# CarluerJB/3D_SIFT_CUDA

Measured on AMD Instinct MI355X. Metric: keypoints/s (.key records per second; Gauss-pyramid GB/s vs HBM roofline in `pyramid`/`roofline`), higher is better.
Workload: dtype f32; 1 GPU; 512^3 float32 blob-field volume per GPU, full featExtract path (pyramid + DoG + extrema + keypoints + SIFT-rank descriptor), all octaves; records_per_volume=185421, octaves=8, extrema=43900, keypoints=36792, parallelism=single GPU, tuning=defaults, descriptor_parity=SIFT-rank: pinned against the reference (see DESIGN.md section 2)

## Files before the change

3d_sift_cuda_amd/csrc/api_slab.hip:

```cpp
#include <algorithm>
#include <chrono>
#include <cmath>
#include <cstdarg>
#include <cstdio>
#include <cstdlib>
#include <cstring>
#include <vector>

#include "sift3d_internal.h"

#include "pipeline.h"

extern "C" int sift3d_candidates_reset(sift3d_ctx *c)
{
    if (!c) return SIFT3D_ERR_ARG;
    HIPCHK(c, hipSetDevice(c->device));
    timing_begin(c);
    return cand_reset(c);
}

extern "C" int sift3d_extrema_append_dev(sift3d_ctx *c, const float *d_prev, const float *d_cur, const float *d_next,
                                         int64_t nx, int64_t ny, int64_t nz_local, int level_id, int64_t z_lo, int64_t z_hi)
{
    if (!c || !d_prev || !d_cur || !d_next) return SIFT3D_ERR_ARG;
// ... 5 lines not shown
    if (rc) return rc;
    rc = cand_append(c, {d_prev, d_cur, d_next, nx, ny, nz_local, (int)z_lo, (int)z_hi, level_id}, cand_where(), true);
    if (rc) return rc;
    return fence_out(c);
}

extern "C" int sift3d_lazy_levels_supported(int64_t nx, int64_t ny, int64_t nz_local, float next_sigma)
{
    float taps[SIFT3D_MAX_TAPS];
    return lazy_shape_ok(nx, ny, nz_local) && sift3d_gauss_taps(next_sigma, 0.01f, taps) == 2 * SIFT3D_FAST_MAX_R + 1 ? 1 : 0;
}

extern "C" int sift3d_extrema_append_lazy_dev(sift3d_ctx *c, const float *d_prev, const float *g_prev_a, const float *g_prev_b,
                                              const float *d_cur, const float *d_next, const float *g_next, float next_sigma,
                                              int64_t nx, int64_t ny, int64_t nz_local, int level_id, int64_t z_lo, int64_t z_hi)
{
    if (!c || !d_cur || (!d_prev && !(g_prev_a && g_prev_b)) || (!d_next && !g_next)) return SIFT3D_ERR_ARG;
    if (nx <= 0 || ny <= 0 || nz_local <= 0 || nx >= (1ll << 31) || ny >= (1ll << 31) || nz_local >= 65538 ||
        nx * ny * nz_local > (int64_t)SIFT3D_KEY_IDX_MASK || level_id < 0 || level_id >= 96)
        return set_err(c, SIFT3D_ERR_ARG, "bad extrema_append arguments");
    float taps[SIFT3D_MAX_TAPS];
    const int ntaps = d_next ? 0 : sift3d_gauss_taps(next_sigma, 0.01f, taps);
    if (((!d_prev || !d_next) && !lazy_shape_ok(nx, ny, nz_local)) || (!d_next && ntaps != 2 * SIFT3D_FAST_MAX_R + 1))
        return set_err(c, SIFT3D_ERR_ARG, "this shape or filter needs stored DoG levels (sift3d_lazy_levels_supported)");
    HIPCHK(c, hipSetDevice(c->device));
    int rc = fence_in(c);
    if (rc) return rc;
    level_job jb = {d_prev ? d_prev : g_prev_a, d_cur, d_next, nx, ny, nz_local, (int)z_lo, (int)z_hi, level_id};
    if (!d_prev) jb.prev_b = g_prev_b;
    if (!d_next) {
        jb.next_ntaps = ntaps;
        for (int q = 0; q < ntaps; q++) jb.next_taps[q] = taps[q];
        jb.next_g = g_next;
    }
    rc = cand_append(c, jb, cand_where(), true);
    if (rc) return rc;
    return fence_out(c);
}

static int levels_from_desc(sift3d_ctx *c, const sift3d_level_desc *ld, int n, std::vector<sift3d_level> &levels)
{
    if (!ld || n <= 0 || n > 96) return set_err(c, SIFT3D_ERR_ARG, "bad level table");
    levels.resize((size_t)n);
    for (int i = 0; i < n; i++) {
        sift3d_level &lv = levels[(size_t)i];
        lv.img = ld[i].img;
        lv.XP = (int)ld[i].nx;
        lv.dogc = ld[i].dogc;
        lv.X = (int)ld[i].nx; lv.Y = (int)ld[i].ny; lv.Z = (int)ld[i].nz_global;
        lv.Zl = (int)ld[i].nz_local;
        lv.z_off = (int)ld[i].z_offset;
        lv.sigma_h = ld[i].sigma_h; lv.sigma_c = ld[i].sigma_c; lv.sigma_l = ld[i].sigma_l;
        lv.octave_factor = ld[i].octave_factor;
        lv.pad = 0;
    }
    return SIFT3D_OK;
}

extern "C" int sift3d_candidates_dev(sift3d_ctx *c, const sift3d_level_desc *levels, int n_levels, sift3d_candidate **out,
                                     int64_t *n_out)
{
    if (!c || !out || !n_out) return SIFT3D_ERR_ARG;
    HIPCHK(c, hipSetDevice(c->device));
    std::vector<sift3d_level> lv;
    int rc = levels_from_desc(c, levels, n_levels, lv);
    if (rc) return rc;
    rc = fence_in(c);
    if (rc) return rc;
    int64_t ncand = 0;
    rc = cand_finalize(c, &ncand);
    if (rc) return rc;
    return candidates_to_host(c, lv, ncand, out, n_out);
}

extern "C" int sift3d_describe_dev(sift3d_ctx *c, const sift3d_level_desc *levels, int n_levels, int desc_mode,
                                   float eig_thres, float size_factor, const sift3d_feature **view, const int32_t **group_view,
                                   int64_t *n_out)
{
    if (!c || !view || !n_out) return SIFT3D_ERR_ARG;
    if (desc_mode < SIFT3D_DESC_SIFT || desc_mode > SIFT3D_DESC_NRRIEF) return set_err(c, SIFT3D_ERR_ARG, "bad descriptor mode");
    HIPCHK(c, hipSetDevice(c->device));
    std::vector<sift3d_level> lv;
    int rc = levels_from_desc(c, levels, n_levels, lv);
    if (rc) return rc;
    rc = fence_in(c);
    if (rc) return rc;
    int64_t ncand = 0;
    rc = cand_finalize(c, &ncand);
    if (rc) return rc;
    c->last.n_extrema = ncand;
    rc = describe_sorted(c, lv, ncand, desc_mode, eig_thres, size_factor, n_out);
    if (rc) return rc;
    *view = c->h_recs;
    if (group_view) *group_view = c->h_group;
    return SIFT3D_OK;
}

extern "C" int sift3d_describe_dev_counts(sift3d_ctx *c, const sift3d_level_desc *levels, int n_levels, int desc_mode, float eig_thres,
                                          float size_factor, const int32_t **group_counts, int64_t *n_records)
{
    if (!c || !group_counts || !n_records) return SIFT3D_ERR_ARG;
    if (desc_mode < SIFT3D_DESC_SIFT || desc_mode > SIFT3D_DESC_NRRIEF) return set_err(c, SIFT3D_ERR_ARG, "bad descriptor mode");
    HIPCHK(c, hipSetDevice(c->device));
    std::vector<sift3d_level> lv;
    int rc = levels_from_desc(c, levels, n_levels, lv);
    if (rc) return rc;
    rc = fence_in(c);
// ... 99 lines not shown
```

3d_sift_cuda_amd/csrc/desc_bins.h:

```cpp
#ifndef DESC_BINS_H
#define DESC_BINS_H

#if defined(__HIPCC__) || defined(__CUDACC__)
#define DESC_BINS_HD __host__ __device__
#else
#define DESC_BINS_HD
#endif
#if defined(__clang__)
#define DESC_BINS_UNROLL _Pragma("unroll")
#define DESC_BINS_ROLLED _Pragma("nounroll")
#else
#define DESC_BINS_UNROLL
#define DESC_BINS_ROLLED
#endif

#define DESC_BINS_PD 11
#define DESC_BINS_NI 9
#define DESC_BINS_NINT 729
#define DESC_BINS_BOX 5
#define DESC_BINS_NONE 8
#define DESC_BINS_ZS 83
#define DESC_BINS_LEN (DESC_BINS_NI * DESC_BINS_ZS)

DESC_BINS_HD constexpr float desc_bins_floor_ce(float x) { return (float)(int)x > x ? (float)((int)x - 1) : (float)(int)x; }

DESC_BINS_HD constexpr void interp_coord(float fX, float fMin, float fMax, int &ix, float &w)
{
    if (fX < fMin + 0.5f) {
        ix = (int)fMin;
        w = 1.0f;
    } else if (fX >= fMax - 0.5f) {
        ix = (int)(fMax - 2);
        w = 0.0f;
    } else {
        float mh = fX - 0.5f;
        ix = (int)(__builtin_is_constant_evaluated() ? desc_bins_floor_ce(mh) : __builtin_floorf(mh));
        w = 1.0f - (mh - ((float)ix));
    }
}

DESC_BINS_HD constexpr float desc_bins_weight(int b, int c)
{
    const float binsz = DESC_BINS_PD / (float)2;
    float v = (int)(c / binsz) + 0.5f;
    if ((int)((c + 0) / binsz) != (int)((c + 1) / binsz)) {
        float p0 = ((c + 0) / binsz);
        float p1 = ((c + 1) / binsz);
        v = (p0 + p1) / 2.0f;
    }
    float w = 0;
    int i0 = 0;
    interp_coord(v, 0, 2.0f, i0, w);
    return b ? 1.0f - w : w;
}
static_assert(desc_bins_weight(0, 1) == 1 && desc_bins_weight(0, 2) == 1 && desc_bins_weight(0, 3) == 1 && desc_bins_weight(0, 4) == 1 &&
                  desc_bins_weight(1, 1) == 0 && desc_bins_weight(1, 2) == 0 && desc_bins_weight(1, 3) == 0 && desc_bins_weight(1, 4) == 0,
              "patch coordinates 1 .. 4 belong to bin 0 alone");
static_assert(desc_bins_weight(0, 5) == 0.5f && desc_bins_weight(1, 5) == 0.5f, "the centre plane is shared in halves");
static_assert(desc_bins_weight(0, 6) == 0 && desc_bins_weight(0, 7) == 0 && desc_bins_weight(0, 8) == 0 && desc_bins_weight(0, 9) == 0 &&
                  desc_bins_weight(1, 6) == 1 && desc_bins_weight(1, 7) == 1 && desc_bins_weight(1, 8) == 1 && desc_bins_weight(1, 9) == 1,
              "patch coordinates 6 .. 9 belong to bin 1 alone");

DESC_BINS_HD constexpr int desc_bins_octant(int lane) { return lane & 7; }
DESC_BINS_HD constexpr int desc_bins_axis_bin(int lane, int axis) { return (lane >> (3 + axis)) & 1; }
DESC_BINS_HD constexpr int desc_bins_origin(int b) { return b ? DESC_BINS_BOX : 1; }
DESC_BINS_HD constexpr int desc_bins_entry(int x, int y, int z) { return (z - 1) * DESC_BINS_ZS + (y - 1) * DESC_BINS_NI + (x - 1); }

DESC_BINS_HD constexpr bool desc_bins_needs_all(float mg) { return mg == __builtin_huge_valf(); }

DESC_BINS_HD inline void desc_bins_box_weights(int b, float *w)
{
    DESC_BINS_UNROLL
    for (int d = 0; d < DESC_BINS_BOX; d++) w[d] = b ? desc_bins_weight(1, desc_bins_origin(1) + d) : desc_bins_weight(0, desc_bins_origin(0) + d);
}

DESC_BINS_HD inline float desc_bins_walk(const float *mag, const unsigned char *bin, int lane)
{
    const int o = desc_bins_octant(lane);
    const int bx = desc_bins_axis_bin(lane, 0), by = desc_bins_axis_bin(lane, 1), bz = desc_bins_axis_bin(lane, 2);
    float wx[DESC_BINS_BOX], wy[DESC_BINS_BOX], wz[DESC_BINS_BOX];
    desc_bins_box_weights(bx, wx);
    desc_bins_box_weights(by, wy);
    desc_bins_box_weights(bz, wz);
    const int base = desc_bins_entry(desc_bins_origin(bx), desc_bins_origin(by), desc_bins_origin(bz));
    mag += base;
    bin += base;
    float acc = 0;
    DESC_BINS_UNROLL
    for (int dz = 0; dz < DESC_BINS_BOX; dz++) {
        DESC_BINS_UNROLL
        for (int dy = 0; dy < DESC_BINS_BOX; dy++) {
// ... 30 lines not shown
```

3d_sift_cuda_amd/csrc/kernels_keypoint.hip:

```cpp
#include <cstddef>
#include <type_traits>

#include "desc_bins.h"
#include "sift3d_internal.h"

#define PD SIFT3D_PATCH_DIM
#define PV SIFT3D_PATCH_VOX



__device__ __forceinline__ float trilinear(const float *__restrict__ img, int X, int XP, int Y, int Z, int Zl, int z_off,
                                           float x, float y, float z)
{
    float wx, wy, wz;
    int ix, iy, iz;
    interp_coord(x, 0, (float)X, ix, wx);
    interp_coord(y, 0, (float)Y, iy, wy);
    interp_coord(z, 0, (float)Z, iz, wz);
    iz -= z_off;
    iz = iz < 0 ? 0 : (iz > Zl - 2 ? Zl - 2 : iz);
    const long long XY = (long long)XP * Y;
    const float *p = img + (long long)iz * XY + (long long)iy * XP + ix;
    typedef float f2u __attribute__((ext_vector_type(2), aligned(4)));
    const f2u q00 = *reinterpret_cast<const f2u *>(p), q10 = *reinterpret_cast<const f2u *>(p + XP);
    const f2u q01 = *reinterpret_cast<const f2u *>(p + XY), q11 = *reinterpret_cast<const f2u *>(p + XY + XP);
    const float f000 = q00.x, f100 = q00.y, f010 = q10.x, f110 = q10.y;
    const float f001 = q01.x, f101 = q01.y, f011 = q11.x, f111 = q11.y;
    float fn00 = wx * f000 + (1.0f - wx) * f100;
    float fn01 = wx * f001 + (1.0f - wx) * f101;
    float fn10 = wx * f010 + (1.0f - wx) * f110;
    float fn11 = wx * f011 + (1.0f - wx) * f111;
    float fnn0 = wy * fn00 + (1.0f - wy) * fn10;
    float fnn1 = wy * fn01 + (1.0f - wy) * fn11;
    return wz * fnn0 + (1.0f - wz) * fnn1;
}

__device__ __forceinline__ double finddet(double a1, double a2, double a3, double b1, double b2, double b3, double c1,
                                          double c2, double c3)
{
    return ((a1 * b2 * c3) - (a1 * b3 * c2) - (a2 * b1 * c3) + (a3 * b1 * c2) + (a2 * b3 * c1) - (a3 * b2 * c1));
}
__device__ __forceinline__ double interp_quadratic(double x0, double x1, double x2, double fx0, double fx1, double fx2)
{
    if (!(fx1 < fx0 && fx1 < fx2) && !(fx1 > fx0 && fx1 > fx2)) return x1;
    double a1 = x0 * x0, b1 = x0, c1 = 1;
    double a2 = x1 * x1, b2 = x1, c2 = 1;
    double a3 = x2 * x2, b3 = x2, c3 = 1;
    double d1 = fx0, d2 = fx1, d3 = fx2;
    double det = finddet(a1, a2, a3, b1, b2, b3, c1, c2, c3);
    double detx = finddet(d1, d2, d3, b1, b2, b3, c1, c2, c3);
    double dety = finddet(a1, a2, a3, d1, d2, d3, c1, c2, c3);
    if (d1 == 0 && d2 == 0 && d3 == 0) return x1;
    if (det != 0) {
        if (detx != 0) return dety / (-2.0 * detx);
    }
    return x1;
}

__device__ __forceinline__ void invert3(const float *in, float *out)
{
    float a11 = in[0], a21 = in[3], a31 = in[6];
    float a12 = in[1], a22 = in[4], a32 = in[7];
    float a13 = in[2], a23 = in[5], a33 = in[8];
    float det = a11 * (a33 * a22 - a32 * a23) - a21 * (a33 * a12 - a32 * a13) + a31 * (a23 * a12 - a22 * a13);
    double div = 1 / (double)det;
    out[0] = (float)((a33 * a22 - a32 * a23) * div);
    out[3] = (float)(-(a33 * a21 - a31 * a23) * div);
    out[6] = (float)((a32 * a21 - a31 * a22) * div);
    out[1] = (float)(-(a33 * a12 - a32 * a13) * div);
    out[4] = (float)((a33 * a11 - a31 * a13) * div);
    out[7] = (float)(-(a32 * a11 - a31 * a12) * div);
    out[2] = (float)((a23 * a12 - a22 * a13) * div);
    out[5] = (float)(-(a23 * a11 - a21 * a13) * div);
    out[8] = (float)((a22 * a11 - a21 * a12) * div);
}

__device__ __forceinline__ void v3_norm(float *p)
{
// ... 172 lines not shown
                c = f / z;
                s = h / z;
                f = x * c + g * s;
                g = g * c - x * s;
                h = y * s;
                y *= c;
                for (int r = 0; r < 3; r++) {
                    x = v[r][j];
                    z = v[r][i];
                    v[r][j] = (float)(x * c + z * s);
                    v[r][i] = (float)(z * c - x * s);
                }
                z = svd_hypot(f, h);
                w[j] = (float)z;
                if (z) {
                    z = 1.0 / z;
                    c = f * z;
                    s = h * z;
                }
                f = c * g + s * y;
                x = c * y - s * g;
                for (int r = 0; r < 3; r++) {
                    y = a[r][j];
                    z = a[r][i];
                    a[r][j] = (float)(y * c + z * s);
                    a[r][i] = (float)(z * c - y * s);
                }
            }
            off[lo] = 0.0;
            off[k] = f;
            w[k] = (float)x;
        }
    }
}
__device__ __forceinline__ void sort_eig(float w[3], float v[3][3])
{
    float t;
    for (int i = 0; i < 3; i++)
        for (int j = i + 1; j < 3; j++)
            if (w[i] < w[j]) {
                t = w[j]; w[j] = w[i]; w[i] = t;
                for (int k = 0; k < 3; k++) {
                    t = v[k][j]; v[k][j] = v[k][i]; v[k][i] = t;
                }
            }
}
typedef float v4f __attribute__((ext_vector_type(4)));
#define KP_NT 256
#define DESC_NT 128
#define NRAD 515
#define NRAD_PAD 516
#define NINT 729

template <int NT>
__device__ __forceinline__ void wave_sample_patch(float *patch, const float *__restrict__ img, int X, int XP, int Y, int Z, int Zl,
                                                  int z_off, float fx, float fy, float fz, float scale, const float *ori9)
{
    float inv[9];
    invert3(ori9, inv);
    const float rad = 2.0f * scale;
    const int sr = PD / 2;
    const float sc = rad / (float)(sr);
    int ax_fast = 0, ax_mid = 1, ax_slow = 2;
    {
        const float f0 = fabsf(inv[0]), f1 = fabsf(inv[1]), f2 = fabsf(inv[2]);
        ax_fast = f0 >= f1 && f0 >= f2 ? 0 : (f1 >= f2 ? 1 : 2);
        const int r0 = ax_fast == 0 ? 1 : 0, r1 = ax_fast == 2 ? 1 : 2;
        const bool first = fabsf(inv[3 + r0]) >= fabsf(inv[3 + r1]);
        ax_mid = first ? r0 : r1;
        ax_slow = first ? r1 : r0;
    }
    const int st_fast = ax_fast == 0 ? 1 : (ax_fast == 1 ? PD : PD * PD), st_mid = ax_mid == 0 ? 1 : (ax_mid == 1 ? PD : PD * PD),
              st_slow = ax_slow == 0 ? 1 : (ax_slow == 1 ? PD : PD * PD);
    for (int s0 = threadIdx.x; s0 < PV; s0 += 3 * NT) {
        float pix[3];
        int sidx[3];
#pragma unroll
        for (int u = 0; u < 3; u++) {
            const int t = s0 + NT * u;
            pix[u] = 0;
            sidx[u] = 0;
            if (t < PV) {
                const int s = (t % PD) * st_fast + ((t / PD) % PD) * st_mid + (t / (PD * PD)) * st_slow;
                sidx[u] = s;
                const int xx = s % PD - sr, yy = (s / PD) % PD - sr, zz = s / (PD * PD) - sr;
                float in3[3] = {(float)xx, (float)yy, (float)zz};
                float o[3];
#pragma unroll
                for (int i = 0; i < 3; i++) {
                    float a = 0;
#pragma unroll
                    for (int j = 0; j < 3; j++) a += inv[i * 3 + j] * in3[j];
                    o[i] = a;
                }
                o[0] *= sc; o[1] *= sc; o[2] *= sc;
                o[0] += fx; o[1] += fy; o[2] += fz;
                if (o[0] < 0 || o[0] >= X) pix[u] = 0;
                else pix[u] = trilinear(img, X, XP, Y, Z, Zl, z_off, o[0], o[1], o[2]);
            }
        }
#pragma unroll
        for (int u = 0; u < 3; u++)
            if (s0 + NT * u < PV) patch[sidx[u]] = pix[u];
    }
    __syncthreads();
}

template <bool SQUARE>
__device__ __forceinline__ float serial_sum_patch(const float *d)
{
    float acc = 0;
    const v4f *d4 = reinterpret_cast<const v4f *>(d);
    v4f a[8], b[8];
    auto add_block = [&](const v4f(&blk)[8]) {
#pragma unroll
        for (int q = 0; q < 8; q++) {
            const v4f v = blk[q];
            if (SQUARE) {
                acc += v.x * v.x; acc += v.y * v.y; acc += v.z * v.z; acc += v.w * v.w;
            } else {
                acc += v.x; acc += v.y; acc += v.z; acc += v.w;
            }
        }
    };
#pragma unroll
    for (int q = 0; q < 8; q++) a[q] = d4[q];
    for (int blk = 0; blk + 1 < 41; blk += 2) {
#pragma unroll
        for (int q = 0; q < 8; q++) b[q] = d4[(blk + 1) * 8 + q];
        add_block(a);
#pragma unroll
        for (int q = 0; q < 8; q++) a[q] = d4[(blk + 2) * 8 + q];
        add_block(b);
    }
    add_block(a);
    for (int i = 41 * 32; i < PV; i++) acc += SQUARE ? d[i] * d[i] : d[i];
    return acc;
}

template <int NT>
__device__ __forceinline__ void wave_normalize_patch(float *d, float *scratch2)
{
    if (threadIdx.x == 0) scratch2[0] = serial_sum_patch<false>(d) / (PD * PD * PD);
    __syncthreads();
    const float mean = scratch2[0];
    for (int i = threadIdx.x; i < PV; i += NT) d[i] -= mean;
    __syncthreads();
    if (threadIdx.x == 0) scratch2[1] = 1.0f / sqrtf(serial_sum_patch<true>(d));
    __syncthreads();
    const float div = scratch2[1];
    for (int i = threadIdx.x; i < PV; i += NT) d[i] *= div;
    __syncthreads();
}

__device__ __forceinline__ bool in_radius(int s)
{
    const int x = s % PD - PD / 2, y = (s / PD) % PD - PD / 2, z = s / (PD * PD) - PD / 2;
    const float fx = (float)x, fy = (float)y, fz = (float)z;
    return fz * fz + fy * fy + fx * fx < (float)((PD / 2) * (PD / 2));
}

__device__ __forceinline__ int wave_build_radius_list(unsigned short *rlist, int *n_lds)
{
    if (threadIdx.x < 64) {
        int n = 0;
        for (int base = 0; base < PV; base += 64) {
            const int s = base + threadIdx.x;
            const bool in = s < PV && in_radius(s);
            const unsigned long long m = __ballot(in);
            if (in) rlist[n + __popcll(m & ((1ull << threadIdx.x) - 1ull))] = (unsigned short)s;
            n += __popcll(m);
        }
        if (threadIdx.x == 0) *n_lds = n;
    }
    __syncthreads();
    return *n_lds;
}

template <int NT>
__device__ __forceinline__ void blur_pass(const float *src, float *dst, int axis, const float *taps, int ntaps)
{
    const int h = ntaps / 2;
    const int st = axis == 0 ? 1 : (axis == 1 ? PD : PD * PD);
    float tp[5], w[5];
#pragma unroll
    for (int j = 0; j < 5; j++) tp[j] = j < ntaps ? taps[j] : 0.0f;
    for (int ln = threadIdx.x; ln < PD * PD; ln += NT) {
        const int base = axis == 0 ? ln * PD : (axis == 1 ? (ln / PD) * PD * PD + ln % PD : ln);
#pragma unroll
        for (int j = 0; j < 5; j++) {
            const int pos = j - h;
            w[j] = (j < ntaps && pos >= 0 && pos < PD) ? src[base + pos * st] : 0.0f;
        }
#pragma unroll
        for (int c = 0; c < PD; c++) {
            float acc = 0;
#pragma unroll
            for (int j = 0; j < 5; j++) {
                const int cc = c + j - h;
                if (j < ntaps && cc >= 0 && cc < PD) acc = acc + tp[j] * w[j];
            }
// ... 173 lines not shown
    float gx[NRAD_PAD], gy[NRAD_PAD], gz[NRAD_PAD];
    union {
        unsigned short rlist[NRAD_PAD];
        short sp_base[NRAD_PAD];
    } r;
    short pk_idx[128];
    float pk_val[128];
    float ori_data[PD * 3 + 3];
    float sc[16];
    float taps[8];
    int cnt[4];
};
static_assert(sizeof(kpA_smem) * 7 <= 160 * 1024, "seven workgroups per CU");
static_assert(offsetof(kpA_smem, C) == sizeof(float) * (PV + 1) && sizeof(float) * (PV + 1) + sizeof(float) * 2 * NRAD_PAD >= 16 * NRAD_PAD,
              "the splat parameters span A and C");

__global__ __launch_bounds__(KP_NT, 7) void keypoint_kernel(sift3d_kp_params p, const unsigned long long *__restrict__ keys,
                                                      const sift3d_cval *__restrict__ vals, long long ncand,
                                                      sift3d_dkp *__restrict__ kps, int *__restrict__ nrec_out,
                                                      sift3d_taps taps3)
{
    __shared__ __attribute__((aligned(16))) kpA_smem sm;
    const long long k = blockIdx.x;
    if (k >= ncand) return;
    const int lane = threadIdx.x;
    if (lane < 3) sm.taps[lane] = taps3.f[lane];
    const unsigned long long key = keys[k];
    const sift3d_cval cvl = vals[k];
    const int lvl = (int)(key >> SIFT3D_KEY_LVL_SHIFT);
    const int is_max = (int)((key >> SIFT3D_KEY_MAX_SHIFT) & 1ull);
    const long long cidx = (long long)(key & SIFT3D_KEY_IDX_MASK);
    const sift3d_level lv = p.levels[lvl];
    sift3d_dkp *kp = kps + k;
    const int X = lv.X, Y = lv.Y, Z = lv.Z, XP = lv.XP;
    const long long XY = (long long)XP * Y;
    const int ix = (int)(cidx % XP), iy = (int)((cidx / XP) % Y), iz = (int)(cidx / XY) + lv.z_off;

    const float *C = lv.dogc;
    const float cv = C[cidx];
    float fx = (float)interp_quadratic(ix - 1, ix, ix + 1, C[cidx - 1], cv, C[cidx + 1]);
    float fy = (float)interp_quadratic(iy - 1, iy, iy + 1, C[cidx - XP], cv, C[cidx + XP]);
    float fz = (float)interp_quadratic(iz - 1, iz, iz + 1, C[cidx - XY], cv, C[cidx + XY]);
    float scale = (float)(2 * interp_quadratic(lv.sigma_h, lv.sigma_c, lv.sigma_l, cvl.h, cv, cvl.l));
    fx += 0.5f; fy += 0.5f; fz += 0.5f;

    const float rad = 2.0f * scale;
    const int rmax = (int)(rad + 2);
    if (fx - rmax < 0 || fy - rmax < 0 || fz - rmax < 0 || fx + rmax >= X || fy + rmax >= Y || fz + rmax >= Z) {
        if (lane == 0) nrec_out[k] = 0;
        return;
    }
    float *patch = sm.A;
    const float ident[9] = {1, 0, 0, 0, 1, 0, 0, 0, 1};
    wave_sample_patch<KP_NT>(patch, lv.img, X, lv.XP, Y, Z, lv.Zl, lv.z_off, fx, fy, fz, scale, ident);
#ifdef SIFT3D_DEV
    if (p.debug_stop == 1) { if (lane == 0) nrec_out[k] = 0; return; }
#endif
    wave_normalize_patch<KP_NT>(patch, sm.sc);
#ifdef SIFT3D_DEV
    if (p.debug_stop == 2) { if (lane == 0) nrec_out[k] = 0; return; }
#endif
    const int nrad = wave_build_radius_list(sm.r.rlist, &sm.cnt[0]);

    for (int i = lane; i < NRAD_PAD; i += KP_NT) {
        float a = 0, b = 0, c = 0;
        if (i < nrad) {
            const int s = sm.r.rlist[i];
            a = patch[s + 1] - patch[s - 1];
            b = patch[s + PD] - patch[s - PD];
            c = patch[s + PD * PD] - patch[s - PD * PD];
        }
        sm.gx[i] = a; sm.gy[i] = b; sm.gz[i] = c;
    }
    __syncthreads();
    if (lane < 9) {
        const float *ei = lane / 3 == 0 ? sm.gx : (lane / 3 == 1 ? sm.gy : sm.gz);
        const float *ej = lane % 3 == 0 ? sm.gx : (lane % 3 == 1 ? sm.gy : sm.gz);
        float acc = 0;
        int i = 0;
        for (; i + 16 <= nrad; i += 16) {
            v4f a[4], b[4];
#pragma unroll
            for (int q = 0; q < 4; q++) {
                a[q] = *reinterpret_cast<const v4f *>(ei + i + 4 * q);
                b[q] = *reinterpret_cast<const v4f *>(ej + i + 4 * q);
            }
#pragma unroll
            for (int q = 0; q < 4; q++) {
                acc += a[q].x * b[q].x; acc += a[q].y * b[q].y; acc += a[q].z * b[q].z; acc += a[q].w * b[q].w;
            }
        }
        for (; i < nrad; i++) acc += ei[i] * ej[i];
        sm.sc[lane] = acc;
    }
    __syncthreads();
#ifdef SIFT3D_DEV
    if (p.debug_stop == 3) { if (lane == 0) nrec_out[k] = 0; return; }
#endif
    auto svd_and_eigen_test = [&]() {
        float mat[3][3], w[3], v[3][3];
        for (int i = 0; i < 3; i++)
            for (int j = 0; j < 3; j++) {
                mat[i][j] = sm.sc[i * 3 + j];
                v[i][j] = 0;
            }
        w[0] = w[1] = w[2] = 0;
        svd3(mat, w, v);
        sort_eig(w, v);
        float es = w[0] + w[1] + w[2];
        float ep = w[0] * w[1] * w[2];
        float esp = es * es * es;
// ... 120 lines not shown
        const int npk2 = wave_peaks_sorted<KP_NT>(ta, sm.C.pk.flags, &sm.cnt[2], sm.C.pk.raw_idx, sm.C.pk.raw_val, sm.C.pk.pk2_idx, sm.C.pk.pk2_val);
#ifdef SIFT3D_DEV
        if (p.debug_stop == 34) { if (lane == 0) nrec_out[k] = 0; return; }
#endif
        const float pk20 = npk2 > 0 ? sm.C.pk.pk2_val[0] : 0.0f;
        for (int j = 0; j < npk2 && nret < PD && nret < 30; j++) {
            if (sm.C.pk.pk2_val[j] < 0.5f * pk20) break;
            if (lane == 0) {
                float p2[3], p3[3];
                interp_point_patch(ta, sm.C.pk.pk2_idx[j], p2);
                p2[0] -= radius; p2[1] -= radius; p2[2] -= radius;
                v3_norm(p2);
                float par = v3_dot(p1, p2);
                p2[0] = p2[0] - par * p1[0];
                p2[1] = p2[1] - par * p1[1];
                p2[2] = p2[2] - par * p1[2];
                v3_norm(p2);
                p3[0] = p1[1] * p2[2] - p1[2] * p2[1];
                p3[1] = -p1[0] * p2[2] + p1[2] * p2[0];
                p3[2] = p1[0] * p2[1] - p1[1] * p2[0];
                float *m = kp->frames + 9 * nret;
                for (int iv = 0; iv < 3; iv++) {
                    m[0 * 3 + iv] = p1[iv];
                    m[1 * 3 + iv] = p2[iv];
                    m[2 * 3 + iv] = p3[iv];
                }
            }
            nret++;
        }
    }
    if (lane == 0) {
        kp->nframes = nret;
        nrec_out[k] = 1 + nret;
    }
}

__device__ __forceinline__ float lane_value(float x, int i)
{
    return __builtin_bit_cast(float, __builtin_amdgcn_readlane(__builtin_bit_cast(int, x), i));
}

__constant__ unsigned char c_brief_x[192] = {
    5,4,4,4,4,2,6,5,5,4,4,4,3,8,5,5,6,3,5,5,5,5,6,5,4,6,6,6,3,4,4,4,5,3,4,5,4,5,5,4,2,7,7,5,3,5,4,5,3,5,7,3,5,5,2,3,5,5,6,6,4,6,5,4,
    4,6,5,3,5,6,4,3,6,4,4,5,3,3,3,6,6,5,2,4,4,6,3,6,3,2,3,5,4,5,3,4,3,6,5,4,3,6,4,5,2,4,3,7,2,3,6,5,2,6,3,3,5,6,3,6,3,5,3,6,5,7,4,2,
    5,5,5,2,5,7,4,2,5,3,4,3,3,7,4,4,7,6,4,4,2,8,7,6,5,4,7,3,6,6,5,2,4,5,3,2,5,5,1,6,3,6,3,6,2,5,4,4,7,2,6,3,2,2,4,3,3,2,3,4,2,5,6,7};
__constant__ unsigned char c_brief_y[192] = {
    6,5,3,4,5,3,7,4,6,4,3,2,4,7,5,3,5,1,5,4,7,6,8,4,4,5,6,5,2,5,4,6,4,0,4,3,3,4,4,2,1,7,8,6,4,4,1,6,1,3,7,2,3,3,1,3,6,1,6,6,4,7,6,4,
    3,5,4,2,3,6,4,5,6,3,3,5,1,3,1,6,7,4,1,4,3,5,2,4,2,1,2,5,4,5,2,3,3,3,3,4,2,6,3,4,3,3,3,6,1,2,5,4,2,4,1,4,6,7,3,6,2,4,3,6,5,6,4,0,
    6,6,5,1,4,7,2,1,5,3,4,2,2,7,3,3,6,4,2,4,1,9,7,7,5,2,7,1,7,5,5,1,5,4,1,3,3,4,0,5,1,6,3,5,3,2,3,3,7,2,5,1,1,0,4,1,3,1,0,3,1,6,5,9};

struct kpB_sift {
    float mag[DESC_BINS_LEN];
    unsigned char bin[DESC_BINS_LEN + 1];
    int hold[379];
    int all;
};
struct kpB_brief {
    float t1[PV + 1];
};
template <bool SIFT>
struct kpB_smem {
    float patch[PV + 1];
    struct {
        typename std::conditional<SIFT, kpB_sift, kpB_brief>::type v;
    } u;
    float sc[16];
    float taps[8];
};

static_assert(sizeof(kpB_smem<true>) > 160 * 1024 / 16 && sizeof(kpB_smem<true>) <= 160 * 1024 / 15 && sizeof(kpB_smem<false>) > 160 * 1024 / 16 &&
                  sizeof(kpB_smem<false>) <= 160 * 1024 / 15,
              "15 records per CU by LDS (160 KB)");

template <bool SIFT>
__global__ __launch_bounds__(DESC_NT) void descriptor_kernel(sift3d_kp_params p, const sift3d_dkp *__restrict__ kps,
                                                        const int *__restrict__ rec_kp, const int *__restrict__ rec_frame,
                                                        long long nrec, sift3d_feature *__restrict__ recs,
                                                        int *__restrict__ rec_group, sift3d_taps taps5)
{
    __shared__ __attribute__((aligned(16))) kpB_smem<SIFT> sm;
    const long long r = xcd_contiguous_item(nrec, p.desc_seg);
    if (r >= nrec) return;
    const int lane = threadIdx.x;
    if (lane < 5) sm.taps[lane] = taps5.f[lane];
    if constexpr (SIFT) {
        if (lane == 5) sm.u.v.all = 0;
    }
    const sift3d_dkp *kp = kps + rec_kp[r];
    const int fr = rec_frame[r];
    float ori[9];
    if (fr < 0) {
        ori[0] = 1; ori[1] = 0; ori[2] = 0; ori[3] = 0; ori[4] = 1; ori[5] = 0; ori[6] = 0; ori[7] = 0; ori[8] = 1;
    } else {
        for (int i = 0; i < 9; i++) ori[i] = kp->frames[fr * 9 + i];
    }
    const sift3d_level lv = p.levels[kp->lvl];
#ifdef SIFT3D_DEV
    if (p.debug_stop >= 21 && p.debug_stop <= 26) {
        wave_sample_patch<DESC_NT>(sm.patch, lv.img, lv.X, lv.XP, lv.Y, lv.Z, lv.Zl, lv.z_off, 20.0f, 20.0f, 20.0f, 3.0f, ori);
        if (p.debug_stop == 21) return;
    } else
#endif
    if (fr < 0) {
        const float *src = p.patch0 + (long long)rec_kp[r] * PV;
        for (int s = lane; s < PV; s += DESC_NT) sm.patch[s] = src[s];
        __syncthreads();
    } else {
        int *tok = nullptr;
        if (p.sampler_cap > 0) {
            unsigned hw, xcc;
            asm volatile("s_getreg_b32 %0, hwreg(HW_REG_HW_ID)" : "=s"(hw));
            asm volatile("s_getreg_b32 %0, hwreg(HW_REG_XCC_ID)" : "=s"(xcc));
            tok = p.sampler_tokens + ((((xcc & 7u) * 8u + ((hw >> 13) & 7u)) * 2u + ((hw >> 12) & 1u)) * 16u + ((hw >> 8) & 15u));
            if (lane == 0) {
                for (int tries = 0;; tries++) {
                    if (atomicAdd(tok, 1) < p.sampler_cap || tries > 50000) break;
                    atomicSub(tok, 1);
                    __builtin_amdgcn_s_sleep(64);
                }
            }
            __syncthreads();
        }
        wave_sample_patch<DESC_NT>(sm.patch, lv.img, lv.X, lv.XP, lv.Y, lv.Z, lv.Zl, lv.z_off, kp->x, kp->y, kp->z, kp->scale, ori);
        if (tok && lane == 0) atomicSub(tok, 1);
    }
#ifdef SIFT3D_DEV
    if (p.debug_stop == 11) return;
#endif
    wave_normalize_patch<DESC_NT>(sm.patch, sm.sc);
#ifdef SIFT3D_DEV
    if (p.debug_stop == 12 || p.debug_stop == 23) return;
#endif

    const bool w0 = lane < 64;
    float myval = 0.0f;
    if constexpr (SIFT) {
        for (int q = lane; q < NINT; q += DESC_NT) {
            const int x = q % 9 + 1, y = (q / 9) % 9 + 1, z = q / 81 + 1;
            const int s = (z * PD + y) * PD + x;
            float e[3] = {sm.patch[s + 1] - sm.patch[s - 1], sm.patch[s + PD] - sm.patch[s - PD],
                          sm.patch[s + PD * PD] - sm.patch[s - PD * PD]};
            float mg = v3_mag(e);
            int best = 8;
            if (mg > 0) {
                v3_norm(e);
                const float oa[8][3] = {{1, 1, 1},  {1, 1, -1},  {1, -1, 1},  {1, -1, -1},
                                        {-1, 1, 1}, {-1, 1, -1}, {-1, -1, 1}, {-1, -1, -1}};
                best = 0;
                float bd = v3_dot(oa[0], e);
#pragma unroll
                for (int t = 1; t < 8; t++) {
                    float d = v3_dot(oa[t], e);
                    if (d > bd) {
                        bd = d;
                        best = t;
                    }
                }
            }
            const int en = desc_bins_entry(x, y, z);
            sm.u.v.mag[en] = mg;
            sm.u.v.bin[en] = (unsigned char)best;
            if (desc_bins_needs_all(mg)) sm.u.v.all = 1;
        }
        __syncthreads();
#ifdef SIFT3D_DEV
        if (p.debug_stop == 13 || p.debug_stop == 24) return;
#endif
        if (w0) {
            const float acc = sm.u.v.all ? desc_bins_walk_all(sm.u.v.mag, sm.u.v.bin, lane) : desc_bins_walk(sm.u.v.mag, sm.u.v.bin, lane);
#ifdef SIFT3D_DEV
            if (p.debug_stop == 26) return;
#endif
            float mn = 100000;
#pragma unroll
            for (int i = 0; i < 64; i++) {
                float vi = lane_value(acc, i);
                if (vi < mn) mn = vi;
            }
            float v = acc - mn;
            float ss = 0;
#pragma unroll
            for (int i = 0; i < 64; i++) {
                float vi = lane_value(v, i);
                ss += vi * vi;
            }
            float div = 1.0f / sqrtf(ss);
            myval = v * div;
        }
    } else {
        wave_blur_patch<DESC_NT>(sm.patch, sm.u.v.t1, sm.patch, sm.taps, 5);
        if (w0) {
            const float *bl = sm.u.v.t1;
            const int x1 = c_brief_x[3 * lane], y1 = c_brief_x[3 * lane + 1], z1 = c_brief_x[3 * lane + 2];
            const int x2 = c_brief_y[3 * lane], y2 = c_brief_y[3 * lane + 1], z2 = c_brief_y[3 * lane + 2];
            float d = bl[x1 + y1 * PD + z1 * PD * PD] - bl[x2 + y2 * PD + z2 * PD * PD];
            if (p.desc_mode == SIFT3D_DESC_BRIEF) {
                myval = (d < 0) ? 1.0f : 0.0f;
            } else if (p.desc_mode == SIFT3D_DESC_RRIEF) {
                myval = d;
            } else {
                float fdx = x1 - x2, fdy = y1 - y2, fdz = z1 - z2;
                int dist = (int)sqrtf(fdx * fdx + fdy * fdy + fdz * fdz);
                myval = d / dist;
            }
        }
    }
    if (!w0) return;
    int rank = 0;
    const unsigned long long nans = __ballot(myval != myval);
    if (nans == 0) {
#pragma unroll
        for (int j = 0; j < 64; j++) {
            float vj = lane_value(myval, j);
            rank += (vj < myval || (vj == myval && j < lane)) ? 1 : 0;
        }
    } else {
        const unsigned long long below = nans & ((1ull << lane) - 1ull), above = lane == 63 ? 0ull : nans & ~((2ull << lane) - 1ull);
        const int lo = below ? 64 - __clzll((long long)below) : 0;
        const int hi = above ? __ffsll((long long)above) - 1 : 64;
        rank = lo;
        for (int j = 0; j < 64; j++) {
            float vj = lane_value(myval, j);
// ... 99 lines not shown
```

3d_sift_cuda_amd/csrc/pipeline.h:

```cpp
#ifndef SIFT3D_PIPELINE_H
#define SIFT3D_PIPELINE_H
#include <cmath>
#include <cstdint>
#include <cstring>
#include <vector>

#include "sift3d_internal.h"

#define SIFT3D_KP_MAX_CHUNKS 16
#define SIFT3D_KP_DEFAULT_CHUNKS 1
#define SIFT3D_D4TINY_FLOATS 32768

struct timed_launch {
    int stage;
    hipEvent_t e0, e1;
    int ntaps;
    int64_t nvox;
    double bytes;
    float ms;
    float start_ms;
};

struct level_job {
    const float *dp, *dc, *dn;
// ... 12 lines not shown
};

struct octave_sigmas {
    float extra0;
    float extras[5];
    float sig[6];
};
static inline octave_sigmas sigma_schedule(float initial_image_scale)
{
    octave_sigmas s;
    float sigma_init = 0.5f;
    if (initial_image_scale > 0) sigma_init /= initial_image_scale;
    const float factor = (float)pow(2.0, 1.0 / (double)3);
    s.extra0 = sqrtf(1.6f * 1.6f - sigma_init * sigma_init);
    float sg = 1.6f;
    s.sig[0] = sg;
    for (int j = 0; j < 5; j++) {
        s.extras[j] = sg * sqrtf(factor * factor - 1.0f);
        sg *= factor;
        s.sig[j + 1] = sg;
    }
    return s;
}

static inline void octave_jobs(level_job jobs[3], const float *const L[5], const float *const D[5], int64_t XP, int64_t Xl, int64_t Y,
                               int64_t Zl, int z_lo, int z_hi, int first_id, const float *next_taps, int next_ntaps)
{
    for (int l = 0; l < 3; l++) jobs[l] = {D[l], D[l + 1], D[l + 2], XP, Y, Zl, z_lo, z_hi, first_id + l, Xl};
    if (!D[0]) {
        jobs[0].dp = L[0];
        jobs[0].prev_b = L[1];
    }
    if (!D[4]) {
        jobs[2].next_g = L[4];
        jobs[2].next_ntaps = next_ntaps;
        for (int q = 0; q < next_ntaps; q++) jobs[2].next_taps[q] = next_taps[q];
    }
}

static inline void octave_level_rows(sift3d_level rows[3], const float *const L[5], const float *const D[5], int64_t X, int64_t XP, int64_t Y,
                                     int64_t Z, int64_t Zl, int64_t z_off, const octave_sigmas &s, float octave_factor)
{
    for (int l = 0; l < 3; l++) {
        sift3d_level &lv = rows[l];
        memset(&lv, 0, sizeof lv);
        lv.img = L[l + 1];
        lv.dogc = D[l + 1];
        lv.X = (int)X; lv.Y = (int)Y; lv.Z = (int)Z;
        lv.XP = (int)XP;
        lv.sigma_h = s.sig[l]; lv.sigma_c = s.sig[l + 1]; lv.sigma_l = s.sig[l + 2];
        lv.octave_factor = octave_factor;
        lv.Zl = (int)Zl;
        lv.z_off = (int)z_off;
    }
}

struct octave_run {
    bool tiny_done;
    bool lazy;
    float *d4tiny;
};

struct sift3d_ctx {
    int device;
    hipStream_t stream;
    hipStream_t ex_stream;
    hipStream_t ex_stream2;
    hipEvent_t ev_ex2[2];
    hipEvent_t ev_reset;
    sift3d_survivor *surv2;
    int64_t surv2_cap;
    hipStream_t kp_stream;
    hipEvent_t ev_kpc[SIFT3D_KP_MAX_CHUNKS];
    hipEvent_t ev_desc;
    hipEvent_t ev_split[3];
    unsigned long long *h_cnt0;
    hipEvent_t ev_oct[2];
    hipEvent_t ev_fence[2];
    bool own_stream;
    int64_t capN;
    int64_t capTot;
    float *vol;
    float *L[6];
    float *D[5];
    float *D4tiny;
    float *T[2];
    float *d_taps;
    unsigned long long *keys_a, *keys_b;
    sift3d_cval *vals_a, *vals_b;
    int64_t cand_cap;
    unsigned long long *d_count;
    int64_t cand_split_at;
    sift3d_survivor *surv;
    sift3d_survivor2 *list2[2];
    int64_t list2_cap[2];
    unsigned long long *list2_counts;
    unsigned long long *surv_counts;
    int surv_set;
    int64_t surv_cap;
    int surv_div;
    void *sort_tmp;
    size_t sort_tmp_bytes;
    void *scan_tmp;
    size_t scan_tmp_bytes;
    sift3d_level *d_levels;
    sift3d_dkp *kps;
// ... 185 lines not shown
```

3d_sift_cuda_amd/csrc/sift3d_internal.h:

```cpp
#ifndef SIFT3D_INTERNAL_H
#define SIFT3D_INTERNAL_H

#include <hip/hip_runtime.h>
#include <stdint.h>

#include "blur_plan.h"
#include "extrema_plan.h"
#include "sift3d.h"
#include "sift3d_dev.h"

#define SIFT3D_MAX_TAPS 129
#define SIFT3D_FAST_MAX_R 8
#define SIFT3D_PATCH_DIM 11
#define SIFT3D_PATCH_VOX 1331

struct sift3d_taps {
    float f[2 * SIFT3D_FAST_MAX_R + 1];
};

typedef float v4f __attribute__((ext_vector_type(4)));
template <int VEC>
struct vecT;
template <> struct vecT<4> { typedef v4f type; };
template <> struct vecT<1> { typedef float type; };
template <int VEC>
__device__ __forceinline__ typename vecT<VEC>::type vload(const float *p)
{
    return *reinterpret_cast<const typename vecT<VEC>::type *>(p);
}
template <int VEC>
__device__ __forceinline__ void vstore(float *p, typename vecT<VEC>::type v)
{
    *reinterpret_cast<typename vecT<VEC>::type *>(p) = v;
}

#define SIFT3D_KEY_LVL_SHIFT 40
#define SIFT3D_KEY_MAX_SHIFT 39
#define SIFT3D_KEY_IDX_MASK ((1ull << 39) - 1ull)
struct sift3d_survivor {
    long long idx;
    float value;
    int is_max;
};
struct sift3d_survivor2 {
    int x, y, z;
    int is_max;
    float value;
    float h;
};
struct sift3d_cval {
    float value, h, l, pad;
};

struct sift3d_level {
    const float *img;
    const float *dogc;
    int X, Y, Z;
    int XP;
    float sigma_h, sigma_c, sigma_l;
    float octave_factor;
    int Zl;
    int z_off;
    int pad;
};

hipError_t sift3d_launch_blur_x(hipStream_t s, const float *in, float *out, int64_t X, int64_t Y, int64_t Z,
                                const float *taps, int ntaps, const float *d_taps);
hipError_t sift3d_launch_blur_y(hipStream_t s, const float *in, float *out, int64_t X, int64_t Y, int64_t Z,
                                const float *taps, int ntaps, const float *d_taps);
hipError_t sift3d_launch_blur_z(hipStream_t s, const float *in, float *out, const float *prev, float *dog, int64_t X,
                                int64_t Y, int64_t Z, const float *taps, int ntaps, const float *d_taps);
hipError_t sift3d_launch_blur_fused(hipStream_t s, const float *in, float *out, float *dog, int64_t X, int64_t Y, int64_t Z,
                                    const float *taps, int ntaps, const sift3d_blur_tuning &tune, int64_t zo0 = 0, int64_t zo1 = -1,
                                    float *sub = nullptr, int *sub_done = nullptr);
hipError_t sift3d_launch_dog(hipStream_t s, const float *a, const float *b, float *out, int64_t n);
hipError_t sift3d_launch_subsample(hipStream_t s, const float *in, int64_t X, int64_t Xl, int64_t Y, int64_t Z, float *out,
                                   int64_t XPout);
hipError_t sift3d_launch_zero_pad(hipStream_t s, float *a, float *b, int64_t X, int64_t Xl, int64_t rows);
#define SIFT3D_TINY_VOX 4096
#define SIFT3D_EAGER_T_FLOATS (1ll << 31)
struct sift3d_octave_out {
    float *L[5];
    float *D[5];
};
struct sift3d_octave_taps {
    float f[5][2 * SIFT3D_FAST_MAX_R + 1];
    int n[5];
};
hipError_t sift3d_launch_tiny_octave(hipStream_t s, const float *L0, const sift3d_octave_out &o, int64_t X, int64_t XP, int64_t Y,
                                     int64_t Z, const sift3d_octave_taps &t);
hipError_t sift3d_launch_double_size(hipStream_t s, const float *in, int64_t X, int64_t Y, int64_t Z, float *out);
hipError_t sift3d_launch_halve_size(hipStream_t s, const float *in, int64_t X, int64_t Y, int64_t Z, float *out);
struct sift3d_extrema_lazy {
    const float *prev_b;
    const float *next_g;
    float taps[2 * SIFT3D_FAST_MAX_R + 1];
    int ntaps;
    sift3d_survivor2 *list2;
    unsigned long long *list2_count;
    int64_t list2_cap;
};
static_assert(EX_LAZY_NTAPS == 2 * SIFT3D_FAST_MAX_R + 1, "the third phase is built for the widest filter of the templated kernels");
struct cand_target {
    unsigned long long *keys;
    sift3d_cval *vals;
    unsigned long long *count;
    int64_t cap;
};
struct sift3d_extrema_pass {
    const float *dprev, *dcur, *dnext;
    int64_t X, Xl, Y, Z;
    int z_lo, z_hi, lvl_id;
    cand_target out;
    sift3d_survivor *surv;
    unsigned long long *surv_count;
    unsigned long long *surv_overflow;
    int64_t surv_cap;
// ... 80 lines not shown
```

Before: 20.63 million keypoints/s.

## Use 32-bit offsets for trilinear gathers and streamline patch sampling and normalization

Adds a per-level off32 flag, set when the level fits in 2 GB, so trilinear sampling computes byte offsets in 32-bit unsigned arithmetic on global address-space pointers instead of 64-bit indexing. interp_coord is replaced with a branch-free select form, patch index mapping is computed directly from per-axis coordinates, and normalization writes squared deviations into a shared buffer so both reductions use one sum routine. The descriptor shared-memory layout moves the 'all' flag out and overlays the squared buffer in a union. The aim is fewer VALU instructions, lower register pressure and less divergence in the keypoint and descriptor kernels, at the cost of a runtime branch on the flag and extra shared-memory writes.

After: 20.87 million keypoints/s (median of 6 runs). 1.2% higher.

```diff
diff --git a/3d_sift_cuda_amd/csrc/api_slab.hip b/3d_sift_cuda_amd/csrc/api_slab.hip
--- a/3d_sift_cuda_amd/csrc/api_slab.hip
+++ b/3d_sift_cuda_amd/csrc/api_slab.hip
@@ -81,7 +81,7 @@
         lv.z_off = (int)ld[i].z_offset;
         lv.sigma_h = ld[i].sigma_h; lv.sigma_c = ld[i].sigma_c; lv.sigma_l = ld[i].sigma_l;
         lv.octave_factor = ld[i].octave_factor;
-        lv.pad = 0;
+        lv.off32 = sift3d_level_off32(ld[i].nx, ld[i].ny, ld[i].nz_local);
     }
     return SIFT3D_OK;
 }
diff --git a/3d_sift_cuda_amd/csrc/desc_bins.h b/3d_sift_cuda_amd/csrc/desc_bins.h
--- a/3d_sift_cuda_amd/csrc/desc_bins.h
+++ b/3d_sift_cuda_amd/csrc/desc_bins.h
@@ -37,6 +37,17 @@
         ix = (int)(__builtin_is_constant_evaluated() ? desc_bins_floor_ce(mh) : __builtin_floorf(mh));
         w = 1.0f - (mh - ((float)ix));
     }
+}
+
+DESC_BINS_HD inline void interp_coord_select(float fX, float fMin, float fMax, int &ix, float &w)
+{
+    const bool low = fX < fMin + 0.5f;
+    const bool high = !low && fX >= fMax - 0.5f;
+    const float mh = ((low || high) ? fMin + 0.5f : fX) - 0.5f;
+    const int im = (int)__builtin_floorf(mh);
+    const float wm = 1.0f - (mh - ((float)im));
+    ix = low ? (int)fMin : (high ? (int)(fMax - 2) : im);
+    w = low ? 1.0f : (high ? 0.0f : wm);
 }
 
 DESC_BINS_HD constexpr float desc_bins_weight(int b, int c)
diff --git a/3d_sift_cuda_amd/csrc/kernels_keypoint.hip b/3d_sift_cuda_amd/csrc/kernels_keypoint.hip
--- a/3d_sift_cuda_amd/csrc/kernels_keypoint.hip
+++ b/3d_sift_cuda_amd/csrc/kernels_keypoint.hip
@@ -9,21 +9,37 @@
 
 
 
+template <bool OFF32>
 __device__ __forceinline__ float trilinear(const float *__restrict__ img, int X, int XP, int Y, int Z, int Zl, int z_off,
                                            float x, float y, float z)
 {
     float wx, wy, wz;
     int ix, iy, iz;
-    interp_coord(x, 0, (float)X, ix, wx);
-    interp_coord(y, 0, (float)Y, iy, wy);
-    interp_coord(z, 0, (float)Z, iz, wz);
+    interp_coord_select(x, 0, (float)X, ix, wx);
+    interp_coord_select(y, 0, (float)Y, iy, wy);
+    interp_coord_select(z, 0, (float)Z, iz, wz);
     iz -= z_off;
     iz = iz < 0 ? 0 : (iz > Zl - 2 ? Zl - 2 : iz);
-    const long long XY = (long long)XP * Y;
-    const float *p = img + (long long)iz * XY + (long long)iy * XP + ix;
     typedef float f2u __attribute__((ext_vector_type(2), aligned(4)));
-    const f2u q00 = *reinterpret_cast<const f2u *>(p), q10 = *reinterpret_cast<const f2u *>(p + XP);
-    const f2u q01 = *reinterpret_cast<const f2u *>(p + XY), q11 = *reinterpret_cast<const f2u *>(p + XY + XP);
+    f2u q00, q10, q01, q11;
+    if constexpr (OFF32) {
+        typedef const __attribute__((address_space(1))) char *gbytes;
+        typedef const __attribute__((address_space(1))) f2u *gpair;
+        const gbytes base = (gbytes)img;
+        const unsigned row = (unsigned)XP * 4u, plane = row * (unsigned)Y;
+        const unsigned b = (unsigned)iz * plane + (unsigned)iy * row + (unsigned)ix * 4u;
+        q00 = *(gpair)(base + b);
+        q10 = *(gpair)(base + (b + row));
+        q01 = *(gpair)(base + (b + plane));
+        q11 = *(gpair)(base + (b + plane + row));
+    } else {
+        const long long XY = (long long)XP * Y;
+        const float *p = img + (long long)iz * XY + (long long)iy * XP + ix;
+        q00 = *reinterpret_cast<const f2u *>(p);
+        q10 = *reinterpret_cast<const f2u *>(p + XP);
+        q01 = *reinterpret_cast<const f2u *>(p + XY);
+        q11 = *reinterpret_cast<const f2u *>(p + XY + XP);
+    }
     const float f000 = q00.x, f100 = q00.y, f010 = q10.x, f110 = q10.y;
     const float f001 = q01.x, f101 = q01.y, f011 = q11.x, f111 = q11.y;
     float fn00 = wx * f000 + (1.0f - wx) * f100;
@@ -302,26 +318,23 @@
 #define NRAD_PAD 516
 #define NINT 729
 
-template <int NT>
-__device__ __forceinline__ void wave_sample_patch(float *patch, const float *__restrict__ img, int X, int XP, int Y, int Z, int Zl,
-                                                  int z_off, float fx, float fy, float fz, float scale, const float *ori9)
+template <int NT, bool OFF32>
+__device__ __forceinline__ void wave_sample_patch_as(float *patch, const float *__restrict__ img, int X, int XP, int Y, int Z, int Zl,
+                                                     int z_off, float fx, float fy, float fz, float scale, const float *ori9)
 {
     float inv[9];
     invert3(ori9, inv);
     const float rad = 2.0f * scale;
     const int sr = PD / 2;
     const float sc = rad / (float)(sr);
-    int ax_fast = 0, ax_mid = 1, ax_slow = 2;
+    int ax_fast = 0, ax_mid = 1;
     {
         const float f0 = fabsf(inv[0]), f1 = fabsf(inv[1]), f2 = fabsf(inv[2]);
         ax_fast = f0 >= f1 && f0 >= f2 ? 0 : (f1 >= f2 ? 1 : 2);
         const int r0 = ax_fast == 0 ? 1 : 0, r1 = ax_fast == 2 ? 1 : 2;
         const bool first = fabsf(inv[3 + r0]) >= fabsf(inv[3 + r1]);
         ax_mid = first ? r0 : r1;
-        ax_slow = first ? r1 : r0;
-    }
-    const int st_fast = ax_fast == 0 ? 1 : (ax_fast == 1 ? PD : PD * PD), st_mid = ax_mid == 0 ? 1 : (ax_mid == 1 ? PD : PD * PD),
-              st_slow = ax_slow == 0 ? 1 : (ax_slow == 1 ? PD : PD * PD);
+    }
     for (int s0 = threadIdx.x; s0 < PV; s0 += 3 * NT) {
         float pix[3];
         int sidx[3];
@@ -331,9 +344,12 @@
             pix[u] = 0;
             sidx[u] = 0;
             if (t < PV) {
-                const int s = (t % PD) * st_fast + ((t / PD) % PD) * st_mid + (t / (PD * PD)) * st_slow;
-                sidx[u] = s;
-                const int xx = s % PD - sr, yy = (s / PD) % PD - sr, zz = s / (PD * PD) - sr;
+                const int rows = t / PD, c_fast = t - rows * PD, c_slow = rows / PD, c_mid = rows - c_slow * PD;
+                const int px = ax_fast == 0 ? c_fast : (ax_mid == 0 ? c_mid : c_slow);
+                const int py = ax_fast == 1 ? c_fast : (ax_mid == 1 ? c_mid : c_slow);
+                const int pz = ax_fast == 2 ? c_fast : (ax_mid == 2 ? c_mid : c_slow);
+                sidx[u] = (pz * PD + py) * PD + px;
+                const int xx = px - sr, yy = py - sr, zz = pz - sr;
                 float in3[3] = {(float)xx, (float)yy, (float)zz};
                 float o[3];
 #pragma unroll
@@ -346,7 +362,7 @@
                 o[0] *= sc; o[1] *= sc; o[2] *= sc;
                 o[0] += fx; o[1] += fy; o[2] += fz;
                 if (o[0] < 0 || o[0] >= X) pix[u] = 0;
-                else pix[u] = trilinear(img, X, XP, Y, Z, Zl, z_off, o[0], o[1], o[2]);
+                else pix[u] = trilinear<OFF32>(img, X, XP, Y, Z, Zl, z_off, o[0], o[1], o[2]);
             }
         }
 #pragma unroll
@@ -355,8 +371,13 @@
     }
     __syncthreads();
 }
-
-template <bool SQUARE>
+template <int NT>
+__device__ __forceinline__ void wave_sample_patch(float *patch, const sift3d_level &lv, float fx, float fy, float fz, float scale, const float *ori9)
+{
+    if (lv.off32) wave_sample_patch_as<NT, true>(patch, lv.img, lv.X, lv.XP, lv.Y, lv.Z, lv.Zl, lv.z_off, fx, fy, fz, scale, ori9);
+    else wave_sample_patch_as<NT, false>(patch, lv.img, lv.X, lv.XP, lv.Y, lv.Z, lv.Zl, lv.z_off, fx, fy, fz, scale, ori9);
+}
+
 __device__ __forceinline__ float serial_sum_patch(const float *d)
 {
     float acc = 0;
@@ -366,11 +387,7 @@
 #pragma unroll
         for (int q = 0; q < 8; q++) {
             const v4f v = blk[q];
-            if (SQUARE) {
-                acc += v.x * v.x; acc += v.y * v.y; acc += v.z * v.z; acc += v.w * v.w;
-            } else {
-                acc += v.x; acc += v.y; acc += v.z; acc += v.w;
-            }
+            acc += v.x; acc += v.y; acc += v.z; acc += v.w;
         }
     };
 #pragma unroll
@@ -384,19 +401,23 @@
         add_block(b);
     }
     add_block(a);
-    for (int i = 41 * 32; i < PV; i++) acc += SQUARE ? d[i] * d[i] : d[i];
+    for (int i = 41 * 32; i < PV; i++) acc += d[i];
     return acc;
 }
 
 template <int NT>
-__device__ __forceinline__ void wave_normalize_patch(float *d, float *scratch2)
-{
-    if (threadIdx.x == 0) scratch2[0] = serial_sum_patch<false>(d) / (PD * PD * PD);
+__device__ __forceinline__ void wave_normalize_patch(float *d, float *scratch2, float *sq)
+{
+    if (threadIdx.x == 0) scratch2[0] = serial_sum_patch(d) / (PD * PD * PD);
     __syncthreads();
     const float mean = scratch2[0];
-    for (int i = threadIdx.x; i < PV; i += NT) d[i] -= mean;
-    __syncthreads();
-    if (threadIdx.x == 0) scratch2[1] = 1.0f / sqrtf(serial_sum_patch<true>(d));
+    for (int i = threadIdx.x; i < PV; i += NT) {
+        const float c = d[i] - mean;
+        d[i] = c;
+        sq[i] = c * c;
+    }
+    __syncthreads();
+    if (threadIdx.x == 0) scratch2[1] = 1.0f / sqrtf(serial_sum_patch(sq));
     __syncthreads();
     const float div = scratch2[1];
     for (int i = threadIdx.x; i < PV; i += NT) d[i] *= div;
@@ -676,11 +697,11 @@
     }
     float *patch = sm.A;
     const float ident[9] = {1, 0, 0, 0, 1, 0, 0, 0, 1};
-    wave_sample_patch<KP_NT>(patch, lv.img, X, lv.XP, Y, Z, lv.Zl, lv.z_off, fx, fy, fz, scale, ident);
+    wave_sample_patch<KP_NT>(patch, lv, fx, fy, fz, scale, ident);
 #ifdef SIFT3D_DEV
     if (p.debug_stop == 1) { if (lane == 0) nrec_out[k] = 0; return; }
 #endif
-    wave_normalize_patch<KP_NT>(patch, sm.sc);
+    wave_normalize_patch<KP_NT>(patch, sm.sc, sm.B);
 #ifdef SIFT3D_DEV
     if (p.debug_stop == 2) { if (lane == 0) nrec_out[k] = 0; return; }
 #endif
@@ -907,8 +928,6 @@
 struct kpB_sift {
     float mag[DESC_BINS_LEN];
     unsigned char bin[DESC_BINS_LEN + 1];
-    int hold[379];
-    int all;
 };
 struct kpB_brief {
     float t1[PV + 1];
@@ -916,11 +935,13 @@
 template <bool SIFT>
 struct kpB_smem {
     float patch[PV + 1];
-    struct {
+    union {
         typename std::conditional<SIFT, kpB_sift, kpB_brief>::type v;
+        float sq[PV + 1];
     } u;
     float sc[16];
     float taps[8];
+    int all;
 };
 
 static_assert(sizeof(kpB_smem<true>) > 160 * 1024 / 16 && sizeof(kpB_smem<true>) <= 160 * 1024 / 15 && sizeof(kpB_smem<false>) > 160 * 1024 / 16 &&
@@ -939,7 +960,7 @@
     const int lane = threadIdx.x;
     if (lane < 5) sm.taps[lane] = taps5.f[lane];
     if constexpr (SIFT) {
-        if (lane == 5) sm.u.v.all = 0;
+        if (lane == 5) sm.all = 0;
     }
     const sift3d_dkp *kp = kps + rec_kp[r];
     const int fr = rec_frame[r];
@@ -952,7 +973,7 @@
     const sift3d_level lv = p.levels[kp->lvl];
 #ifdef SIFT3D_DEV
     if (p.debug_stop >= 21 && p.debug_stop <= 26) {
-        wave_sample_patch<DESC_NT>(sm.patch, lv.img, lv.X, lv.XP, lv.Y, lv.Z, lv.Zl, lv.z_off, 20.0f, 20.0f, 20.0f, 3.0f, ori);
+        wave_sample_patch<DESC_NT>(sm.patch, lv, 20.0f, 20.0f, 20.0f, 3.0f, ori);
         if (p.debug_stop == 21) return;
     } else
 #endif
@@ -976,13 +997,13 @@
             }
             __syncthreads();
         }
-        wave_sample_patch<DESC_NT>(sm.patch, lv.img, lv.X, lv.XP, lv.Y, lv.Z, lv.Zl, lv.z_off, kp->x, kp->y, kp->z, kp->scale, ori);
+        wave_sample_patch<DESC_NT>(sm.patch, lv, kp->x, kp->y, kp->z, kp->scale, ori);
         if (tok && lane == 0) atomicSub(tok, 1);
     }
 #ifdef SIFT3D_DEV
     if (p.debug_stop == 11) return;
 #endif
-    wave_normalize_patch<DESC_NT>(sm.patch, sm.sc);
+    wave_normalize_patch<DESC_NT>(sm.patch, sm.sc, sm.u.sq);
 #ifdef SIFT3D_DEV
     if (p.debug_stop == 12 || p.debug_stop == 23) return;
 #endif
@@ -1015,14 +1036,14 @@
             const int en = desc_bins_entry(x, y, z);
             sm.u.v.mag[en] = mg;
             sm.u.v.bin[en] = (unsigned char)best;
-            if (desc_bins_needs_all(mg)) sm.u.v.all = 1;
+            if (desc_bins_needs_all(mg)) sm.all = 1;
         }
         __syncthreads();
 #ifdef SIFT3D_DEV
         if (p.debug_stop == 13 || p.debug_stop == 24) return;
 #endif
         if (w0) {
-            const float acc = sm.u.v.all ? desc_bins_walk_all(sm.u.v.mag, sm.u.v.bin, lane) : desc_bins_walk(sm.u.v.mag, sm.u.v.bin, lane);
+            const float acc = sm.all ? desc_bins_walk_all(sm.u.v.mag, sm.u.v.bin, lane) : desc_bins_walk(sm.u.v.mag, sm.u.v.bin, lane);
 #ifdef SIFT3D_DEV
             if (p.debug_stop == 26) return;
 #endif
diff --git a/3d_sift_cuda_amd/csrc/pipeline.h b/3d_sift_cuda_amd/csrc/pipeline.h
--- a/3d_sift_cuda_amd/csrc/pipeline.h
+++ b/3d_sift_cuda_amd/csrc/pipeline.h
@@ -88,6 +88,7 @@
         lv.octave_factor = octave_factor;
         lv.Zl = (int)Zl;
         lv.z_off = (int)z_off;
+        lv.off32 = sift3d_level_off32(XP, Y, Zl);
     }
 }
 
diff --git a/3d_sift_cuda_amd/csrc/sift3d_internal.h b/3d_sift_cuda_amd/csrc/sift3d_internal.h
--- a/3d_sift_cuda_amd/csrc/sift3d_internal.h
+++ b/3d_sift_cuda_amd/csrc/sift3d_internal.h
@@ -61,8 +61,9 @@
     float octave_factor;
     int Zl;
     int z_off;
-    int pad;
+    int off32;
 };
+static inline int sift3d_level_off32(int64_t XP, int64_t Y, int64_t Zl) { return XP * Y * Zl * (int64_t)sizeof(float) < (1ll << 31) ? 1 : 0; }
 
 hipError_t sift3d_launch_blur_x(hipStream_t s, const float *in, float *out, int64_t X, int64_t Y, int64_t Z,
                                 const float *taps, int ntaps, const float *d_taps);
```
